# dflemin3/approxposterior

Measured on AMD Instinct MI355X. Metric: GP-predict+acquisition candidates/sec (N_train, D fixed), higher is better.
Workload: dtype f64

## Files before the change

approxposterior_amd/_lib.py:

```python
import ctypes
import os

_HERE = os.path.dirname(os.path.abspath(__file__))
LIB_PATH = os.path.join(_HERE, "csrc", "libapgp.so")
ABI_VERSION = 8
MAX_DIM = 32
MAX_FANTASY = 32
MAX_DRAWS = 32
MAX_FEATURES = 65536
MAX_REFS = 4096
INTEGRATED_MAX_DIM = 16

UTIL_AGP, UTIL_BAPE, UTIL_JONES, UTIL_NONE = 0, 1, 2, 3
UTIL_NEG_MEAN = 4
NM_MAX_RESTARTS = 4096
NM_MAX_FEV = 1 << 20
NM_STEPS = {1: "reflect", 2: "expand", 3: "reflect_exp", 4: "contract_out", 5: "contract_in",
            6: "shrink_out", 7: "shrink_in", 8: "maxfev"}
PRUNE_ROWS_SPLIT, PRUNE_ROWS_SIGNED = 0, 1
GMM_EM, GMM_SCORE, GMM_KMEANS = 0, 1, 2
GMM_MAX_COMP = 16
IMP_BLOCK = 256
IMP_MAX_BLOCKS = 2048

# ... 34 lines not shown

class HmcOptions(ctypes.Structure):
    _fields_ = [("eps", ctypes.c_double), ("jitter", ctypes.c_double), ("nleap", ctypes.c_int32),
                ("g_rows", ctypes.c_int32), ("iteration0", ctypes.c_int64), ("mass", ctypes.c_double * MAX_DIM)]

_P = ctypes.c_void_p
_I64 = ctypes.c_int64
_I32 = ctypes.c_int32
_F64 = ctypes.c_double
_KP = ctypes.POINTER(KernelStruct)

SIGNATURES = {
    "apgp_abi_version": (ctypes.c_int, []),
    "apgp_last_error": (ctypes.c_char_p, []),
    "apgp_npad": (_I64, [_I64]),
    "apgp_packed_linv_len": (_I64, [_I64]),
    "apgp_acquire_work_len": (_I64, [_I64, _I64]),
    "apgp_packed_train_len": (_I64, [_I64, _I32]),
    "apgp_trtri_work_len": (_I64, [_I64]),
    "apgp_grad_work_len": (_I64, [_I64]),
    "apgp_gram": (ctypes.c_int, [_P, _I64, _KP, _P, _I64, _P]),
    "apgp_kernel_cross": (ctypes.c_int, [_P, _I64, _P, _I64, _KP, _P, _I64, _P]),
    "apgp_potrf": (ctypes.c_int, [_P, _I64, _I64, _P, _F64, _P, _P, _P]),
    "apgp_logdet": (ctypes.c_int, [_P, _I64, _I64, _P, _P]),
    "apgp_fit_summary": (ctypes.c_int, [_P, _I64, _I64, _P, _P, _P, _P]),
    "apgp_nll_eval": (ctypes.c_int, [_P, _I64, _KP, _P, _F64, _P, _P, _P, _P, _P, _P]),
    "apgp_potrf_mode": (ctypes.c_int, [ctypes.c_int]),
    "apgp_potrf_fallbacks": (_I64, []),
    "apgp_potrf_backoff_skips": (_I64, []),
    "apgp_nll_side_batches": (_I64, []),
    "apgp_nll_eval_batch": (ctypes.c_int, [_P, _I64, _I64, _P, _P, _P, _P, _P, _P, _P, _P, _P]),
    "apgp_trsv": (ctypes.c_int, [_P, _I64, _I64, _P, _F64, ctypes.c_int, _P, _P, _P]),
    "apgp_trsv_ex": (ctypes.c_int, [_P, _I64, _I64, _P, _F64, ctypes.c_int, _P, _P, ctypes.c_int, _P]),
    "apgp_trsv_mode": (ctypes.c_int, [ctypes.c_int]),
    "apgp_append_diag": (ctypes.c_int, [_P, _P, _F64, _P, _I64, _P]),
    "apgp_winv_apply_work_len": (_I64, [_I64]),
    "apgp_winv_apply": (ctypes.c_int, [_P, _I64, _I64, _P, _F64, ctypes.c_int, _P, _P, _P, _P]),
    "apgp_trtri_pack": (ctypes.c_int, [_P, _I64, _I64, _P, _P, _P, _P]),
    "apgp_pack_train": (ctypes.c_int, [_P, _P, _I64, _KP, _P, _P]),
    "apgp_acquire": (ctypes.c_int, [_P, _I64, _I64, _P, _P, _I64, _KP, _F64, _I32,
                                    ctypes.POINTER(_F64), ctypes.POINTER(_F64), _P,
                                    _F64, _F64, _P, _P, _P, _P, _P, _P]),
    "apgp_packed_lsolve_len": (_I64, [_I64]),
    "apgp_pack_lsolve": (ctypes.c_int, [_P, _I64, _I64, _P, _P]),
    "apgp_acquire_solve": (ctypes.c_int, [_P, _I64, _I64, _P, _P, _I64, _KP, _F64, _I32,
                                          ctypes.POINTER(_F64), ctypes.POINTER(_F64), _P,
                                          _F64, _F64, _P, _P, _P, _P, _P, _P]),
    "apgp_set_sweep_prune": (ctypes.c_int, [ctypes.c_int]),
    "apgp_get_sweep_prune": (ctypes.c_int, []),
    "apgp_set_seed_rowsplit": (ctypes.c_int, [ctypes.c_int]),
    "apgp_get_seed_rowsplit": (ctypes.c_int, []),
    "apgp_set_seed_park": (ctypes.c_int, [ctypes.c_int]),
    "apgp_get_seed_park": (ctypes.c_int, []),
    "apgp_set_seed_first": (ctypes.c_int, [ctypes.c_int]),
    "apgp_get_seed_first": (ctypes.c_int, []),
    "apgp_set_seed_parts": (ctypes.c_int, [ctypes.c_int]),
    "apgp_get_seed_parts": (ctypes.c_int, []),
    "apgp_sweep_prune_counts_offset": (_I64, [_I64, _I64]),
    "apgp_sweep_prune_select": (ctypes.c_int, [_P, _I64, _P, _P, _F64, _P, _P]),
    "apgp_prune_bounds": (ctypes.c_int, [_P, _I64, _P, _I64, _KP, _F64, _I32, ctypes.POINTER(_F64), ctypes.POINTER(_F64),
                                         _P, _F64, _F64, ctypes.c_int, _P, _P]),
    "apgp_sweep_prune_seeds": (ctypes.c_int, [_P, _I64, _P, _P, _P]),
    "apgp_prune_rows_len": (_I64, [_I64, _I32]),
    "apgp_pack_prune_rows": (ctypes.c_int, [_P, _I64, _KP, _P, _P]),
    "apgp_acquire_rows": (ctypes.c_int, [_P, _I64, _I64, _P, _P, _I64, _KP, _F64, _I32,
                                         ctypes.POINTER(_F64), ctypes.POINTER(_F64), _P,
                                         _F64, _F64, _P, _P, _P, _P, _P, _P, _P]),
    "apgp_acquire_solve_rows": (ctypes.c_int, [_P, _I64, _I64, _P, _P, _I64, _KP, _F64, _I32,
                                               ctypes.POINTER(_F64), ctypes.POINTER(_F64), _P,
                                               _F64, _F64, _P, _P, _P, _P, _P, _P, _P]),
    "apgp_prune_bounds_rows": (ctypes.c_int, [_P, _I64, _P, _I64, _KP, _F64, _I32, ctypes.POINTER(_F64),
                                              ctypes.POINTER(_F64), _P, _F64, _F64, ctypes.c_int, _P, _P, _P]),
    "apgp_prune_srows_len": (_I64, [_I64, _I32]),
    "apgp_pack_prune_srows": (ctypes.c_int, [_P, _I64, _KP, _P, _P]),
    "apgp_acquire_rows2": (ctypes.c_int, [_P, _I64, _I64, _P, _P, _I64, _KP, _F64, _I32,
                                          ctypes.POINTER(_F64), ctypes.POINTER(_F64), _P,
                                          _F64, _F64, _P, _P, _P, _P, _P, _P, _I32, _P]),
    "apgp_acquire_solve_rows2": (ctypes.c_int, [_P, _I64, _I64, _P, _P, _I64, _KP, _F64, _I32,
                                                ctypes.POINTER(_F64), ctypes.POINTER(_F64), _P,
                                                _F64, _F64, _P, _P, _P, _P, _P, _P, _I32, _P]),
    "apgp_prune_bounds_rows2": (ctypes.c_int, [_P, _I64, _P, _I64, _KP, _F64, _I32, ctypes.POINTER(_F64),
                                               ctypes.POINTER(_F64), _P, _F64, _F64, ctypes.c_int, _P, _P, _I32, _P, _P]),
    "apgp_acquire_fantasy_work_len": (_I64, [_I64]),
    "apgp_acquire_fantasy": (ctypes.c_int, [_P, _I64, _I64, _P, _I64, _KP, _P, _I64, _I32, _P, _I64,
                                            _P, _P, _P, _I32, ctypes.POINTER(_F64), ctypes.POINTER(_F64), _P,
                                            _F64, _F64, _P, _P, _P, _P]),
    "apgp_path_draws_work_len": (_I64, [_I64, _I32]),
    "apgp_path_draws_mode": (ctypes.c_int, [ctypes.c_int]),
    "apgp_path_draws": (ctypes.c_int, [_P, _I64, _I64, _P, _I64, _KP, _F64, _P, _P, _P, _P, _P, _I32, _I32,
                                       ctypes.POINTER(_F64), ctypes.POINTER(_F64), _P, _P, _P, _P, _P]),
    "apgp_integrated_work_len": (_I64, [_I64, _I32]),
    "apgp_integrated_mode": (ctypes.c_int, [ctypes.c_int]),
    "apgp_acquire_integrated": (ctypes.c_int, [_P, _I64, _I64, _P, _I64, _KP, _P, _I32, _P, _P, _P,
                                               ctypes.POINTER(_F64), ctypes.POINTER(_F64), _P, _P, _I64, _P, _P, _P, _P]),
    "apgp_predict1_work_len": (_I64, [_I64]),
    "apgp_predict1_host": (ctypes.c_int, [_P, _P, _I64, _KP, _F64, _P, _I64, _P, _I64, _P, _P, _P]),
    "apgp_nm_search_work_len": (_I64, [_I64, _I64]),
    "apgp_nm_search": (ctypes.c_int, [_P, _I64, _P, _I64, _KP, _F64, _P, _I64, _P, _I64,
                                      ctypes.POINTER(_F64), ctypes.POINTER(_F64), ctypes.POINTER(NmOptions),
                                      _P, _P, _P, _P, _P, _P, _P]),
    "apgp_predict_grad_work_len": (_I64, [_I64, _I64]),
    "apgp_predict_grad": (ctypes.c_int, [_P, _I64, _P, _I64, _KP, _F64, _P, _I64, _P, _I64, _I32,
                                         ctypes.POINTER(_F64), ctypes.POINTER(_F64), _F64, _F64,
                                         _P, _P, _P, _P, _P, _P, _P, _P]),
    "apgp_predict_mean": (ctypes.c_int, [_P, _I64, _P, _I64, _KP, _F64, _P, _P]),
    "apgp_predict_mean_host": (ctypes.c_int, [_P, _I64, _P, _I64, _KP, _F64, _P, _P, _P]),
# ... 78 lines not shown
```

approxposterior_amd/csrc/prune_mm32.h:

```cpp
#pragma once
#include <utility>

#ifndef PMM_G
#define PMM_G 4
#endif
#define PMM_ROWS 128
typedef float f32x16 __attribute__((ext_vector_type(16)));
typedef __bf16 bf16x8 __attribute__((ext_vector_type(8)));

struct PmmSlot { int e, pp, qp; };

template <int DPAD>
struct PmmShape {
    static constexpr int K = DPAD + 2;
    static constexpr int NS = 5 * DPAD + 4;
    static constexpr int NIS = (NS + 15) / 16, NI = NIS + 1;
    static constexpr int PITCH = 16 * NI + 8;
    static_assert(K <= 16, "the big products stand in one instruction");
    static constexpr int XPIECES = PMM_ROWS * PITCH / 8, APIECES = PMM_ROWS / 4, PIECES = XPIECES + APIECES;
    static constexpr PmmSlot slot(int i) {
        if (i >= 16 * NIS) return i - 16 * NIS < K ? PmmSlot{i - 16 * NIS, 0, 0} : PmmSlot{-1, 0, 0};
        if (i < 2 * DPAD) return PmmSlot{2 + i / 2, (i & 1) ? 2 : 0, (i & 1) ? 0 : 2};
        i -= 2 * DPAD;
        if (i < 2) return i == 0 ? PmmSlot{0, 2, 0} : PmmSlot{1, 0, 2};
// ... 153 lines not shown
        for (int j = 0; j < NW; ++j) {
            if (j < w) k += pos ? wp[b][j] : wn[b][j];
            base_p += wp[b][j];
            base_n += wn[b][j];
        }
        k += __popcll((pos ? mp : mn) & below);
        if (in) {
            float pe[DPAD + 2];
            double n2 = 0.0, b2 = 0.0;
#pragma unroll
            for (int d = 0; d < DPAD; ++d) {
                const double x = (d & 1) ? pre[d >> 1].y : pre[d >> 1].x;
                const double df = x - cen[d];
                b2 = fma(df, df, b2);
                const float bf = (float)(df * kappa);
                n2 = fma((double)bf, (double)bf, n2);
                pe[d + 2] = 2.0f * bf;
            }
            bm2 = fmax(bm2, b2);
            sal += fabs(alpha);
            pe[0] = -(float)n2;
            pe[1] = 1.0f;
            const long long r = pmm_srow((pos ? 0 : gp) + (k >> 4), (int)(k & 15));
            pmm_put_row<DPAD>(img + r / PMM_ROWS * (16ll * SH::PIECES), (int)(r % PMM_ROWS), pe, (float)alpha);
        }
    }
    for (long long r = tid; r < pmm_stiles(n) * PMM_ROWS; r += PR_THREADS) {
        const int rr = (int)(r & 31), s = (rr & 3) + 4 * (rr >> 3);
        const long long q = 2 * (r >> 5) + ((rr >> 2) & 1);
        const bool empty = q < gp ? 16 * q + s >= np : q < gp + gn ? 16 * (q - gp) + s >= nn : true;
        if (empty) {
            float pe[DPAD + 2];
#pragma unroll
            for (int d = 0; d < DPAD; ++d) pe[d + 2] = 0.0f;
            pe[0] = -0.0f;
            pe[1] = 1.0f;
            pmm_put_row<DPAD>(img + r / PMM_ROWS * (16ll * SH::PIECES), (int)(r % PMM_ROWS), pe, 0.0f);
        }
    }
    for (int o = 32; o > 0; o >>= 1) { bm2 = fmax(bm2, __shfl_xor(bm2, o)); sal += __shfl_xor(sal, o); }
    if (lane == 0) { wmax[w] = bm2; wsal[w] = sal; }
    __syncthreads();
    if (tid == 0) {
        sal = 0.0;
#pragma unroll
        for (int i = 0; i < NW; ++i) { bm2 = fmax(bm2, wmax[i]); sal += wsal[i]; }
        ((double*)rows)[0] = bm2;
        ((double*)rows)[1] = sal;
        ((long long*)rows)[2] = (gp + gn + 1) / 2;
        ((long long*)rows)[3] = 0;
    }
}

template <int DPAD, bool PRE = false, bool SGN = false>
__global__ __launch_bounds__(PR_THREADS, PMM_G <= 4 ? 2 : 1) void prune_bound_mm32_kernel(PruneArgs a) {
    static_assert(PRE || !SGN, "the sign-sorted rows come as a stream only");
    using SH = PmmShape<DPAD>;
    constexpr int XS = DPAD + 2;
    constexpr int K = SH::K, NI = SH::NI, PITCH = SH::PITCH, G = PMM_G;
    static_assert(PMM_G % 2 == 0 && PMM_ROWS == 32 * (PR_THREADS / 64), "one 32-row tile staged per wavefront");
    const double kappa = PR32_KAPPA;
    static_assert(SH::XPIECES * 8 == PMM_ROWS * PITCH && SH::APIECES * 4 == PMM_ROWS, "the stream's tile is the LDS image");
    constexpr int NB = PRE ? 2 : 1;
    __shared__ __attribute__((aligned(16))) __bf16 xt[NB * PMM_ROWS * PITCH];
    __shared__ __attribute__((aligned(16))) float at[NB * PMM_ROWS];
    __shared__ double wmax[PR_THREADS / 64], wsal[PR_THREADS / 64];
    const int tid = threadIdx.x, lane = tid & 63, w = tid >> 6, h = lane >> 5, l32 = lane & 31;
    const long long blk0 = ((long long)blockIdx.x * (PR_THREADS / 64) + w) * (G / 2);
    double cen[DPAD], c2 = 0.0;
#pragma unroll
    for (int d = 0; d < DPAD; ++d) { cen[d] = a.xs[d]; c2 = fma(cen[d], cen[d], c2); }
    const double cn = sqrt(c2);
    bf16x8 qop[G][NI];
    double an[G];
    bool adm[G];
#pragma unroll
    for (int g = 0; g < G; ++g) {
        const long long blk = blk0 + (g >> 1);
        const long long row = blk * SW_CAND + (g & 1) * 32 + l32;
        const bool live = blk < a.ncb && row < a.m;
        bool ok = live, has_nan = false;
        double a2 = 0.0, ce[DPAD];
#pragma unroll
        for (int d = 0; d < DPAD; ++d) {
            double v = 0.0;
            if (live && d < a.ndim) {
                v = a.T[row * a.ndim + d];
                if (a.has_box && !(v >= a.lo[d] && v <= a.hi[d])) ok = false;
                if (v != v) has_nan = true;
            }
            ce[d] = v * a.sc[d] - cen[d];
            a2 = fma(ce[d], ce[d], a2);
        }
        if (live && a.mask && a.mask[row] == 0) ok = false;
        adm[g] = ok && !has_nan;
        an[g] = sqrt(a2);
        const bool use = live && !has_nan && a2 <= 0x1p100;
        float q[K];
        double n2 = 0.0;
#pragma unroll
        for (int d = 0; d < DPAD; ++d) {
            q[d + 2] = use ? (float)(ce[d] * kappa) : 0.0f;
            n2 = fma((double)q[d + 2], (double)q[d + 2], n2);
        }
        q[0] = 1.0f;
        q[1] = -(float)n2;
        pmm_cand<DPAD>(qop[g], q, h, std::make_integer_sequence<int, NI>{});
    }
    double accm[G], accs[G], sal = 0.0, bm2 = 0.0;
#pragma unroll
    for (int g = 0; g < G; ++g) { accm[g] = 0.0; accs[g] = 0.0; }
    long long nrt = 0;
    if constexpr (SGN) nrt = ((const long long*)a.prune_rows)[2];
    const long long ntile = SGN ? (nrt + PMM_ROWS / 32 - 1) / (PMM_ROWS / 32) : (a.n + PMM_ROWS - 1) / PMM_ROWS;
    auto consume = [&](int xo, int ao, int nr) {
#pragma unroll 1
        for (int rt = 0; rt < (SGN ? nr : PMM_ROWS / 32); ++rt) {
            const __bf16* xr = xt + xo + (rt * 32 + l32) * PITCH + 8 * h;
            bf16x8 pop[NI];
#pragma unroll
            for (int t = 0; t < NI; ++t) pop[t] = *(const bf16x8*)(xr + 16 * t);
            float al[16];
#pragma unroll
            for (int q = 0; q < 4; ++q) *(f32x4*)(al + 4 * q) = *(const f32x4*)(at + ao + rt * 32 + 8 * q + 4 * h);
            auto product = [&](int g) {
                f32x16 c = {0.0f, 0.0f, 0.0f, 0.0f, 0.0f, 0.0f, 0.0f, 0.0f, 0.0f, 0.0f, 0.0f, 0.0f, 0.0f, 0.0f, 0.0f, 0.0f};
#pragma unroll
                for (int t = 0; t < NI; ++t) c = __builtin_amdgcn_mfma_f32_32x32x16_bf16(pop[t], qop[g][t], c, 0, 0, 0);
                return c;
            };
            f32x16 cur = product(0);
#pragma unroll
            for (int g = 0; g < G; ++g) {
                f32x16 nxt = cur;
                if (g + 1 < G) nxt = product(g + 1);
                float ps = 0.0f, pS = 0.0f;
#pragma unroll
                for (int r = 0; r < 16; ++r) {
                    const float k = __builtin_amdgcn_exp2f(cur[r]);
                    ps = fmaf(k, al[r], ps);
                    if constexpr (!SGN) pS = fmaf(k, fabsf(al[r]), pS);
                }
                accm[g] += (double)ps;
                accs[g] += (double)(SGN ? fabsf(ps) : pS);
                cur = nxt;
            }
        }
    };
    if constexpr (PRE) {
        typedef unsigned int u32x4 __attribute__((ext_vector_type(4)));
        constexpr int NPC = SH::PIECES, NL = (NPC + PR_THREADS - 1) / PR_THREADS;
        const u32x4* img = (const u32x4*)((const unsigned char*)a.prune_rows + (SGN ? PMM_SHDR : 16));
        u32x4 pre[NL];
        auto fetch = [&](long long ti) {
            const u32x4* src = img + ti * NPC;
#pragma unroll
            for (int j = 0; j < NL; ++j) {
                const int e = tid + j * PR_THREADS;
                pre[j] = src[e < NPC ? e : NPC - 1];
            }
        };
        auto put = [&](int b) {
            u32x4* xd = (u32x4*)(xt + b * PMM_ROWS * PITCH);
            u32x4* ad = (u32x4*)(at + b * PMM_ROWS);
#pragma unroll
            for (int j = 0; j < NL; ++j) {
                const int e = tid + j * PR_THREADS;
                if ((j + 1) * PR_THREADS <= SH::XPIECES || e < SH::XPIECES) xd[e] = pre[j];
                else if (e < NPC) ad[e - SH::XPIECES] = pre[j];
            }
        };
        fetch(0);
        put(0);
        __syncthreads();
        for (long long ti = 0; ti < ntile; ++ti) {
            const int b = (int)(ti & 1);
            fetch(ti + 1 < ntile ? ti + 1 : ntile - 1);
            const long long left = nrt - ti * (PMM_ROWS / 32);
            consume(b * PMM_ROWS * PITCH, b * PMM_ROWS, left < PMM_ROWS / 32 ? (int)left : PMM_ROWS / 32);
            put(b ^ 1);
            __syncthreads();
        }
        bm2 = ((const double*)a.prune_rows)[0];
        sal = ((const double*)a.prune_rows)[1];
    } else {
        const bool stager = h == 0;
        const int srow = w * 32 + l32;
        f64x2 pre[XS / 2];
        auto fetch = [&](long long ti) {
            const f64x2* src = (const f64x2*)(a.xs + (ti * PMM_ROWS + srow) * XS);
#pragma unroll
            for (int i = 0; i < XS / 2; ++i) pre[i] = stager ? src[i] : f64x2{0.0, 0.0};
        };
        fetch(0);
        for (long long ti = 0; ti < ntile; ++ti) {
            if (stager) {
                const bool in = ti * PMM_ROWS + srow < a.n;
                float pe[K];
                double n2 = 0.0, b2 = 0.0;
#pragma unroll
                for (int d = 0; d < DPAD; ++d) {
                    const double x = (d & 1) ? pre[d >> 1].y : pre[d >> 1].x;
                    const double df = x - cen[d];
                    b2 = fma(df, df, b2);
                    const float bf = in ? (float)(df * kappa) : 0.0f;
                    n2 = fma((double)bf, (double)bf, n2);
                    pe[d + 2] = 2.0f * bf;
                }
                if (in) { bm2 = fmax(bm2, b2); sal += fabs(pre[DPAD / 2].x); }
                pe[0] = -(float)n2;
                pe[1] = 1.0f;
                pmm_store_row<DPAD>(xt + srow * PITCH, pe, std::make_integer_sequence<int, 2 * NI>{});
                at[srow] = in ? (float)pre[DPAD / 2].x : 0.0f;
            }
            __syncthreads();
            if (ti + 1 < ntile) fetch(ti + 1);
            consume(0, 0, PMM_ROWS / 32);
            __syncthreads();
        }
        for (int o = 32; o > 0; o >>= 1) { bm2 = fmax(bm2, __shfl_xor(bm2, o)); sal += __shfl_xor(sal, o); }
        if (lane == 0) { wmax[w] = bm2; wsal[w] = sal; }
        __syncthreads();
        sal = 0.0;
#pragma unroll
        for (int i = 0; i < PR_THREADS / 64; ++i) { bm2 = fmax(bm2, wmax[i]); sal += wsal[i]; }
    }
    const double bn = sqrt(bm2);
    const double u32 = 0x1p-24, eps = 0x1p-53;
    const double sa = sal * (1.0 + 0x1p-16);
    double bb = INFINITY, bbe = INFINITY;
#pragma unroll
    for (int g = 0; g < G; ++g) {
        const double sm = accm[g] + __shfl_xor(accm[g], 32);
// ... 18 lines not shown
```

approxposterior_amd/csrc/sweep.hip:

```cpp
#include "apgp_common.h"
#include "mma16.h"
#include "scratch.h"
#include "util_value.h"
#include <mutex>
#include <stdlib.h>
#include <string.h>

#define SW_ROWS APGP_ROW_BLOCK
#define SW_KC APGP_K_CHUNK
#define SW_TILE (SW_ROWS * SW_KC)
#define SW_CAND 64
#define SW_GRID 256
#define SW_BCH 1024
typedef unsigned int u32x4 __attribute__((ext_vector_type(4)));
#ifndef SW_KAUX
#define SW_KAUX 0
#endif

struct SweepArgs {
    const double* T;
    const double* linv;
    const double* xs;
    const unsigned char* mask;
    double* mu;
// ... 1099 lines not shown
            hipLaunchKernelGGL((sweep2_kernel<DPAD, true, 2, LIST>), dim3(grid), dim3(S2_THREADS), lds, s, a);
        else
            hipLaunchKernelGGL((sweep2_kernel<DPAD, false, 2, LIST>), dim3(grid), dim3(S2_THREADS), lds, s, a);
    } else if (solve) {
        if (a.lin_coef != 0.0)
            hipLaunchKernelGGL((sweep2_kernel<DPAD, true, 1, LIST>), dim3(grid), dim3(S2_THREADS), lds, s, a);
        else
            hipLaunchKernelGGL((sweep2_kernel<DPAD, false, 1, LIST>), dim3(grid), dim3(S2_THREADS), lds, s, a);
    } else if (a.lin_coef != 0.0)
        hipLaunchKernelGGL((sweep2_kernel<DPAD, true, 0, LIST>), dim3(grid), dim3(S2_THREADS), lds, s, a);
    else
        hipLaunchKernelGGL((sweep2_kernel<DPAD, false, 0, LIST>), dim3(grid), dim3(S2_THREADS), lds, s, a);
}

template <int DPAD>
static int launch_sweep(const SweepArgs& a0, hipStream_t s, bool solve) {
    const int rc = s2_prepare_device<DPAD>();
    if (rc != 0) return rc;
    SweepArgs a = a0;
    const long long ncb = (a.m + SW_CAND - 1) / SW_CAND;
    const int nrb2 = s2_nrb(a.n);
    a.nrb = nrb2;
    long long rest = ncb % SW_GRID;
    if (solve || nrb2 < 2 || rest > S2_SPLIT_MAX || a.sp_q == NULL) rest = 0;
    const long long full = ncb - rest;
    if (full > 0) {
        a.blk_begin = 0; a.blk_end = full; a.split = 0;
        s2_launch<DPAD, false>(a, s, solve, (unsigned)(full < SW_GRID ? full : SW_GRID));
    }
    if (rest > 0) {
        a.blk_begin = full; a.blk_end = ncb; a.split = 1;
        a.ncache = 0;
        a.kslot_bytes = SW_BCH * 8;
        s2_launch<DPAD, false>(a, s, solve, (unsigned)(rest * nrb2));
        hipLaunchKernelGGL(sweep_finish_kernel, dim3((unsigned)rest), dim3(64), 0, s, a);
    }
    return 0;
}

static int g_seed_rowsplit = -1;

extern "C" int apgp_set_seed_rowsplit(int v) {
    return __atomic_exchange_n(&g_seed_rowsplit, v < 0 ? -1 : v, __ATOMIC_RELAXED);
}

extern "C" int apgp_get_seed_rowsplit(void) { return __atomic_load_n(&g_seed_rowsplit, __ATOMIC_RELAXED); }

static int g_seed_park = 1;

extern "C" int apgp_set_seed_park(int v) { return __atomic_exchange_n(&g_seed_park, v != 0 ? 1 : 0, __ATOMIC_RELAXED); }

extern "C" int apgp_get_seed_park(void) { return __atomic_load_n(&g_seed_park, __ATOMIC_RELAXED); }

#define S2_SEED_FIRST 4
static int g_seed_first = -1;

extern "C" int apgp_set_seed_first(int v) {
    return __atomic_exchange_n(&g_seed_first, v < 1 ? -1 : (v > 16 ? 16 : v), __ATOMIC_RELAXED);
}

extern "C" int apgp_get_seed_first(void) { return __atomic_load_n(&g_seed_first, __ATOMIC_RELAXED); }

static int g_seed_parts = -1;

extern "C" int apgp_set_seed_parts(int v) {
    return __atomic_exchange_n(&g_seed_parts, (v == 8 || v == 4 || v == 2 || v == 1) ? v : -1, __ATOMIC_RELAXED);
}

extern "C" int apgp_get_seed_parts(void) { return __atomic_load_n(&g_seed_parts, __ATOMIC_RELAXED); }

static long long seed_launch_cost(int nrb, int cap, int n, int j0, int lg, bool parked) {
    static const int gen[4] = {S2P_WHOLE_GEN, S2P_HALF_GEN, S2P_PAIR2_GEN, S2P_PAIR1_GEN};
    static const int park[4] = {S2P_WHOLE_PARK, S2P_HALF_PARK, S2P_PAIR2_PARK, S2P_PAIR1_PARK};
    long long load[SW_GRID] = {0};
    const int nitem = s2_nitems(nrb, j0, n, lg);
    long long last = 0;
    for (int i = 0; i < nitem; ++i) {
        int jb = 0, h = -1;
        s2_row_item(i, nrb, j0, n, lg, jb, h);
        const int kind = h >= 0 ? lg : (n - S2_ROWS * jb <= S2_ROWS / 2 ? 1 : 0);
        const int nkc = s2_nkc_of(jb, n), nre = S2_CPB * jb < nkc ? S2_CPB * jb : nkc;
        const long long c = parked ? (long long)gen[kind] * (nkc - nre) + (long long)park[kind] * nre
                                   : (long long)s2_part_cost(kind) * nkc;
        for (int k = 0; k < cap; ++k) {
            int best = 0;
            for (int q = 1; q < SW_GRID; ++q)
                if (load[q] < load[best]) best = q;
            load[best] += c;
            if (load[best] > last) last = load[best];
        }
    }
    return last;
}

struct SeedPlan { int j0, lg; long long cost; };
static SeedPlan seed_plan(int nrb, int cap, int n, bool parked) {
    const int v = apgp_get_seed_rowsplit(), fp = apgp_get_seed_parts();
    const int flg = fp == 8 ? 0 : fp == 4 ? 1 : fp == 2 ? 2 : fp == 1 ? 3 : -1;
    struct Memo { int nrb, cap, n, parked, v, flg; SeedPlan plan; };
    static std::mutex mu;
    static Memo memo[8];
    static int nmemo = 0, next = 0;
    std::lock_guard<std::mutex> g(mu);
    for (int i = 0; i < nmemo; ++i) {
        const Memo& e = memo[i];
        if (e.nrb == nrb && e.cap == cap && e.n == n && e.parked == (int)parked && e.v == v && e.flg == flg) return e.plan;
// ... 558 lines not shown
    return old;
}

extern "C" int apgp_get_sweep_prune(void) { return __atomic_load_n(&g_sweep_prune, __ATOMIC_RELAXED); }

static inline long long pr_ncb(int64_t m) { return (m + SW_CAND - 1) / SW_CAND; }
static inline long long s2_work_len(int64_t m, int64_t n) {
    const long long ncb = pr_ncb(m);
    const long long slots = ncb < SW_GRID ? ncb : SW_GRID;
    return 2 * ncb + slots * s2_ncache(n) * SW_BCH + 2 * (long long)S2_SPLIT_MAX * SW_CAND * s2_nrb(n);
}

extern "C" int64_t apgp_sweep_prune_counts_offset(int64_t m, int64_t n) {
    if (m < 1 || n < 1 || m > APGP_MAX_M || n > APGP_MAX_N) return -1;
    return s2_work_len(m, n) + 2 * pr_ncb(m) + PR_SEED;
}

extern "C" int apgp_sweep_prune_select(const double* bmin, int64_t ncb, const int64_t* seeds, int64_t* counts,
                                       double tau, int64_t* list, void* stream) {
    APGP_CHECK_ARG(bmin && seeds && counts && list, "null pointer");
    APGP_CHECK_ARG(ncb >= 1 && ncb <= APGP_MAX_M / SW_CAND, "ncb >= 1 required");
    hipLaunchKernelGGL(prune_select_kernel, dim3(1), dim3(1024), 0, (hipStream_t)stream, bmin, (long long)ncb,
                       (const long long*)seeds, (long long*)counts, (const double*)NULL, tau, (long long*)list,
                       (long long*)NULL);
    APGP_CHECK_LAUNCH();
    return 0;
}

static inline bool pr_rows_kind_ok(const void* prune_rows, int rows_kind) {
    return rows_kind == APGP_PRUNE_ROWS_SPLIT || (rows_kind == APGP_PRUNE_ROWS_SIGNED && prune_rows != NULL);
}

template <class Kern>
static PruneArgs pr_args(const double* T, int64_t m, const double* xs, int64_t n, const uint8_t* mask, const Kern& kern,
                         double mean, int32_t kind, const double* lo, const double* hi, double zeta, double ybest,
                         double* bmin, double* part_u, long long* part_i, const void* prune_rows, int rows_kind) {
    PruneArgs p;
    p.T = T; p.xs = xs; p.mask = mask; p.bmin = bmin; p.part_u = part_u; p.part_i = part_i;
    p.m = m; p.ncb = pr_ncb(m); p.n = n;
    p.kind = kind; p.mean = mean; p.zeta = zeta; p.ybest = ybest;
    apgp_fill_kernel(p, kern);
    apgp_fill_box(p, p.ndim, lo, hi);
    p.blk_list = NULL; p.blk_count = NULL; p.est = NULL; p.prune_rows = prune_rows; p.rows_kind = rows_kind;
    return p;
}

template <int DPAD>
static void launch_bound(const PruneArgs& p, hipStream_t s, bool coarse) {
    auto grid_of = [&](int cpt) { return dim3((unsigned)((p.ncb + (PR_THREADS / 64) * cpt - 1) / ((PR_THREADS / 64) * cpt))); };
    const dim3 grid = grid_of(coarse ? pr32_cpt(DPAD) : PR_CPT);
    if (coarse) {
        if constexpr (DPAD <= 8) {
            const dim3 mm_grid = grid_of(PMM_G / 2);
            if (p.prune_rows && p.rows_kind == APGP_PRUNE_ROWS_SIGNED)
                hipLaunchKernelGGL((prune_bound_mm32_kernel<DPAD, true, true>), mm_grid, dim3(PR_THREADS), 0, s, p);
            else if (p.prune_rows)
                hipLaunchKernelGGL((prune_bound_mm32_kernel<DPAD, true>), mm_grid, dim3(PR_THREADS), 0, s, p);
            else
                hipLaunchKernelGGL((prune_bound_mm32_kernel<DPAD, false>), mm_grid, dim3(PR_THREADS), 0, s, p);
            hipLaunchKernelGGL((prune_bound32_kernel<DPAD, true>), grid, dim3(PR_THREADS), 0, s, p);
        } else {
            hipLaunchKernelGGL((prune_bound32_kernel<DPAD, false>), grid, dim3(PR_THREADS), 0, s, p);
        }
    } else if (p.blk_list)
        hipLaunchKernelGGL((prune_bound_kernel<DPAD, true>), grid, dim3(PR_THREADS), 0, s, p);
    else
        hipLaunchKernelGGL((prune_bound_kernel<DPAD, false>), grid, dim3(PR_THREADS), 0, s, p);
}

template <int DPAD>
static int launch_pruned(const SweepArgs& a, hipStream_t s, bool solve, void* part, const void* prune_rows,
                         int rows_kind) {
    const int rc = s2_prepare_device<DPAD>();
    if (rc != 0) return rc;
    const long long ncb = pr_ncb(a.m);
    double* bmin = (double*)part + s2_work_len(a.m, a.n);
    long long* list = (long long*)(bmin + ncb);
    long long* seeds = list + ncb;
    long long* counts = seeds + PR_SEED;
    const bool coarse = a.lin_coef == 0.0;
    PruneArgs p = pr_args(a.T, a.m, a.xs, a.n, a.mask, a, a.mean, a.kind, a.has_box ? a.lo : NULL, a.has_box ? a.hi : NULL,
                          a.zeta, a.ybest, bmin, a.part_u, a.part_i, prune_rows, rows_kind);
    if (coarse) p.est = (double*)(counts + 8);
    launch_bound<DPAD>(p, s, coarse);
    hipLaunchKernelGGL(prune_seed_kernel, dim3(1), dim3(1024), 0, s, coarse ? (const double*)p.est : (const double*)bmin, ncb,
                       seeds, counts);
    if (solve || s2_nrb(a.n) < 2 || a.sp_q == NULL) (void)hipMemsetAsync(counts + 4, 0, sizeof(long long), s);
    launch_sweep_list<DPAD>(a, s, solve, seeds, counts, ncb < PR_SEED ? ncb : PR_SEED, PR_SEED, true);
    hipLaunchKernelGGL(prune_select_kernel, dim3(1), dim3(1024), 0, s, bmin, ncb, seeds, counts, a.part_u, 0.0, list,
                       counts + 3);
    if (coarse) {
        p.blk_list = list; p.blk_count = counts + 3;
        launch_bound<DPAD>(p, s, false);
        hipLaunchKernelGGL(prune_select_kernel, dim3(1), dim3(1024), 0, s, bmin, ncb, seeds, counts, a.part_u, 0.0, list,
                           (long long*)NULL);
    }
    launch_sweep_list<DPAD>(a, s, solve, list, counts + 1, ncb, S2_SPLIT_MAX);
    return 0;
}

static_assert(S2_PRUNE_WORDS == PR_SEED + 8, "the fold inputs start behind the seed numbers and the counters");
static inline long long pr_work_len(int64_t m, int64_t n) {
    return s2_work_len(m, n) - 2ll * S2_SPLIT_MAX * SW_CAND * s2_nrb(n) + s2_fold_off(s2_nrb(n), pr_ncb(m));
}

extern "C" int64_t apgp_acquire_work_len(int64_t m, int64_t n) {
    if (m < 1 || n < 1) return 0;
// ... 566 lines not shown
```

approxposterior_amd/gp.py:

```python

import collections
import ctypes
import math
from operator import is_

import numpy as np
from numpy.linalg import LinAlgError
from scipy.linalg import solve_triangular

from . import _lib
from .george_extras import GeorgeExtras

__all__ = ["GP", "ExpSquaredKernel", "ConstantKernel", "Product", "ConstantModel",
           "kernels", "UTILITY_KINDS", "sobolSample"]

UTILITY_KINDS = {"agp": _lib.UTIL_AGP, "bape": _lib.UTIL_BAPE, "jones": _lib.UTIL_JONES}
SEARCH_KINDS = dict(UTILITY_KINDS, negmean=_lib.UTIL_NEG_MEAN)
NM_OPTIONS = ("adaptive", "maxiter", "maxfev", "xatol", "fatol")


def nm_coefficients(ndim, adaptive):
    if adaptive:
        dim = float(ndim)
        return 1.0, 1 + 2 / dim, 0.75 - 1 / (2 * dim), 1 - 1 / dim
# ... 326 lines not shown
            raise ValueError("Z (R, D), b (R,), W (S, R) and Wl (S, D) do not fit together")
        self.ks = gp._kernel_struct()
        self.mean = float(gp.mean.value)
        self._key, self._x = (gp._factor_key(), self.mean), gp._x

    def _check_current(self):
        gp = self.gp
        if not gp.computed or gp._x is not self._x or (gp._factor_key(), float(gp.mean.value)) != self._key:
            raise RuntimeError("these draws belong to a factor the GP no longer holds: call sample_paths again")

    def _call(self, t, bounds, mask, idx_offset, with_f):
        gp = self.gp
        self._check_current()
        lo, hi = _box(bounds, gp.kernel.ndim)
        T = gp._candidates(t)
        mask_d = mask if hasattr(mask, "data_ptr") else gp._mask(mask, T.shape[0])
        if mask_d is not None and (tuple(mask_d.shape) != (T.shape[0],) or str(mask_d.dtype) != "torch.uint8"):
            raise ValueError("a device mask must be a (M,) uint8 tensor")
        if T.shape[0] == 0:
            return np.empty((self.size, 0)), np.full(self.size, -1, dtype=np.int64), np.full(self.size, np.inf)
        return gp._path_call(T, self.ks, self.mean, self, self.V, lo, hi, mask_d, idx_offset, with_f)

    def evaluate(self, t):
        F = self._call(t, None, None, 0, True)[0]
        return F if isinstance(F, np.ndarray) else F.cpu().numpy()

    def argmax(self, t, bounds=None, mask=None, idx_offset=0):
        _, idx, u = self._call(t, bounds, mask, idx_offset, False)
        return idx, -u



class GP(GeorgeExtras):

    def __init__(self, kernel=None, fit_kernel=True, mean=None, fit_mean=None,
                 white_noise=None, fit_white_noise=None, solver=None, device=None,
                 **kwargs):
        if kernel is None:
            raise ValueError("a kernel is required")
        self.kernel = kernel
        self.mean = _as_model(mean, 0.0)
        self.white_noise = _as_model(white_noise, np.log(1.25e-12))
        self.fit_mean = bool(fit_mean)
        self.fit_white_noise = bool(fit_white_noise)
        self._device_arg = device
        self.variance_mode = None
        self.extend_max_rows = None
        self.sweep_prune = None
        self.seed_rowsplit = None
        self.seed_park = None
        self.seed_first = None
        self.seed_parts = None
        self.prune_signed = True
        self.sweep_prune_stats = False
        self.last_prune_counts = None
        self._computed = False
        self._x = None
        self._yerr2 = 0.0
        self._nllMemo = None
        self._rt_cache = None
        self._queries = None
        self._x_d = None
        self._mean_work = None
        self._p1_work = None
        self._imp_work = None
        self._pimp_work = None
        self._pg_work = None
        self._nll_scratch = None
        self._nll_stream = None
        self._batch = None
        self._replays = {}
        self._reset_device_state()

    def _reset_device_state(self):
        self._L = None
        self._L_store = None
        self._ld = None
        self._nll_owned = False
        self._alpha_y = None
        self._alpha_mean = None
        self._y_d = None
        self._ztz_host = None
        self._z = None
        self._alpha = None
        self._packed = None
        self._packed_solve = None
        self._work = None
        self._xs = None
        self._prune_rows = None
        self._prune_srows = None
        self._xs_key = None
        for key in ("nll", "one", "mean", "pgrad"):
            self._replays.pop(key, None)
        self.cond_estimate = None
        self.log_determinant = None

    def _rt(self):
        if self._rt_cache is not None:
            return self._rt_cache
        import torch
        lib = _lib.load()
        if not torch.cuda.is_available():
            raise _lib.ApgpError("no MI355X visible: approxposterior_amd has no CPU fallback")
        dev = self._device_arg
        if dev is None:
            dev = torch.device("cuda", torch.cuda.current_device())
# ... 691 lines not shown
            p0 = out.data_ptr()
            with_u = kid != _lib.UTIL_NONE
            args = [T.data_ptr(), m, self._xs.data_ptr(), n, ctypes.byref(ks), float(self.mean.value), *inv, kid,
                    lo, hi, float(zeta), float(np.max(y)),
                    p0, p0 + 8 * m, p0 + 16 * m if with_u else None, p0 + 24 * m, p0 + 8 * m * (3 + D),
                    p0 + 8 * m * (3 + 2 * D) if with_u else None, self._pg_work.data_ptr(), st]
            _lib.check(lib.apgp_predict_grad(*args), "apgp_predict_grad")
            if host_point:
                self._replays["pgrad"] = _Replay(
                    lib.apgp_predict_grad, args, dev.index, st.value or 0, y, (self._xs, self._pg_work, factor),
                    self._queries, data=((kid, bkey, float(zeta), self.mean.value), torch, T, out))
            if return_device:
                return self._pgrad_split(out, m, D, kid)
            return self._pgrad_split(out.cpu().numpy(), m, D, kid)

    @staticmethod
    def _pgrad_split(out, m, D, kid):
        mu, var, u = out[:m], out[m:2 * m], out[2 * m:3 * m]
        dmu, dvar, du = (out[m * (3 + j * D):m * (3 + (j + 1) * D)].reshape(m, D) for j in range(3))
        if kid == _lib.UTIL_NONE:
            return mu, var, dmu, dvar
        return u, du, mu, var

    def _sweep(self, y, T, kind_id, lo=None, hi=None, mask_d=None, zeta=0.01, idx_offset=0,
               with_mu=False, with_var=False, with_u=False):
        torch, dev, lib = self._rt()
        y = self._check_dimensions(y)
        n, m = len(self._x), T.shape[0]
        ks = self._kernel_struct()
        use_solve = not self._trust_inverse()
        with self._on(torch, dev):
            st = self._stream(torch)
            if use_solve:
                self._ensure_lsolve()
            else:
                self._ensure_linv()
            self._ensure_xs(y)
            f64 = dict(dtype=torch.float64, device=dev)
            mu, var, u = (torch.empty(m, **f64) if keep else None for keep in (with_mu, with_var, with_u))
            part = torch.empty(max(int(lib.apgp_acquire_work_len(m, n)), 2), **f64)
            best = torch.empty(2, **f64)
            ev = getattr(self, "kernel_events", None)
            if ev is not None:
                e0 = torch.cuda.Event(enable_timing=True)
                e0.record()
            args = (self._xs.data_ptr(), n, ctypes.byref(ks), float(self.mean.value), kind_id, lo, hi, _ptr(mask_d),
                    float(zeta), float(np.max(y)), _ptr(mu), _ptr(var), _ptr(u), part.data_ptr(), best.data_ptr(),
                    *self._prune_stream(), st)
            prune_was = None if self.sweep_prune is None else lib.apgp_set_sweep_prune(int(self.sweep_prune))
            rowsplit_was = None if self.seed_rowsplit is None else lib.apgp_set_seed_rowsplit(int(self.seed_rowsplit))
            park_was = None if self.seed_park is None else lib.apgp_set_seed_park(int(self.seed_park))
            first_was = None if self.seed_first is None else lib.apgp_set_seed_first(int(self.seed_first))
            parts_was = None if self.seed_parts is None else lib.apgp_set_seed_parts(int(self.seed_parts))
            try:
                if use_solve:
                    _lib.check(lib.apgp_acquire_solve_rows2(T.data_ptr(), m, int(idx_offset),
                                                            self._packed_solve.data_ptr(), *args), "apgp_acquire_solve_rows2")
                else:
                    _lib.check(lib.apgp_acquire_rows2(T.data_ptr(), m, int(idx_offset), self._packed.data_ptr(), *args),
                               "apgp_acquire_rows2")
            finally:
                if prune_was is not None:
                    lib.apgp_set_sweep_prune(prune_was)
                if rowsplit_was is not None:
                    lib.apgp_set_seed_rowsplit(rowsplit_was)
                if park_was is not None:
                    lib.apgp_set_seed_park(park_was)
                if first_was is not None:
                    lib.apgp_set_seed_first(first_was)
                if parts_was is not None:
                    lib.apgp_set_seed_parts(parts_was)
            if self.sweep_prune_stats and kind_id != _lib.UTIL_NONE and mu is None and var is None and u is None:
                off = int(lib.apgp_sweep_prune_counts_offset(m, n))
                self.last_prune_counts = part[off:off + 5].view(torch.int64).clone()
            if ev is not None:
                e1 = torch.cuda.Event(enable_timing=True)
                e1.record()
                ev.append((e0, e1))
        return _Swept(best, mu, var, u)

    def acquire(self, y, t, kind, bounds=None, mask=None, zeta=0.01, return_all=False,
                idx_offset=0, device_record=False):
        if not self.computed:
            raise RuntimeError("ERROR: Need to compute GP before using it!")
        kind_id = UTILITY_KINDS[str(kind).lower()]
        if device_record and return_all:
            raise ValueError("device_record returns the arg-min record only")
        torch, dev, _ = self._rt()
        lo, hi = _box(bounds, self.kernel.ndim)
        T = self._candidates(t)
        mask_d = self._mask(mask, T.shape[0])
        y = self._check_dimensions(y)
        if T.shape[0] == 0:
            if device_record:
                return torch.tensor([int(np.float64(np.inf).view(np.int64)), -1], dtype=torch.int64, device=dev)
            return (-1, float("inf")) + ((np.empty(0),) * 3 if return_all else ())
        s = self._sweep(y, T, kind_id, lo, hi, mask_d, zeta, idx_offset, with_mu=return_all, with_var=return_all,
                        with_u=return_all)
        if device_record:
            return s.best.view(torch.int64)
        if not return_all:
            return _best_record(s.best)
        return _best_record(s.best) + (s.u.cpu().numpy(), s.mu.cpu().numpy(), s.var.cpu().numpy())

    def prune_bounds(self, y, t, kind, coarse=True, bounds=None, mask=None, zeta=0.01):
        if not self.computed:
            raise RuntimeError("ERROR: Need to compute GP before using it!")
        kind_id = UTILITY_KINDS[str(kind).lower()]
        torch, dev, lib = self._rt()
        lo, hi = _box(bounds, self.kernel.ndim)
        T = self._candidates(t)
        m = T.shape[0]
        mask_d = self._mask(mask, m)
        y = self._check_dimensions(y)
        ks = self._kernel_struct()
        with self._on(torch, dev):
            self._ensure_xs(y)
            bmin = torch.empty((m + 63) // 64, dtype=torch.float64, device=dev)
            _lib.check(lib.apgp_prune_bounds_rows2(T.data_ptr(), m, self._xs.data_ptr(), len(self._x), ctypes.byref(ks),
                                                   float(self.mean.value), kind_id, lo, hi, _ptr(mask_d), float(zeta),
                                                   float(np.max(y)), int(bool(coarse)), bmin.data_ptr(),
                                                   *self._prune_stream(), None, self._stream(torch)),
                       "apgp_prune_bounds_rows2")
        return bmin.cpu().numpy()

    def nelder_mead_search(self, y, starts, kind, bounds=None, zeta=0.01, options=None, trace=False):
        try:
            kid = SEARCH_KINDS[str(kind).lower()]
        except KeyError:
            raise ValueError("kind must be one of %s" % sorted(SEARCH_KINDS))
        opts = dict(options or {})
        unknown = sorted(set(opts) - set(NM_OPTIONS))
        if unknown:
            raise ValueError("the device Nelder-Mead search does not take the option(s) %s (it takes %s)"
                             % (unknown, ", ".join(NM_OPTIONS)))
        if not self.computed:
            raise RuntimeError("ERROR: Need to compute GP before using it!")
        y = self._check_dimensions(y)
        D = self.kernel.ndim
        lo, hi = _box(bounds, D)
        X0 = np.ascontiguousarray(np.asarray(starts, dtype=np.float64).reshape(-1, D))
        R = len(X0)
        if not 1 <= R <= _lib.NM_MAX_RESTARTS:
            raise ValueError("between 1 and %d restarts per call" % _lib.NM_MAX_RESTARTS)
        rho, chi, psi, sigma = nm_coefficients(D, bool(opts.get("adaptive", False)))
        maxiter, maxfev = nm_limits(D, opts.get("maxiter"), opts.get("maxfev"))
        if not (1 <= maxiter <= _lib.NM_MAX_FEV and 1 <= maxfev <= _lib.NM_MAX_FEV):
            raise ValueError("maxiter and maxfev must lie between 1 and %d" % _lib.NM_MAX_FEV)
        opt = _lib.NmOptions(kind=kid, maxiter=maxiter, maxfev=maxfev, reserved=0, zeta=float(zeta),
                             ybest=float(np.max(y)), xatol=float(opts.get("xatol", 1e-4)),
                             fatol=float(opts.get("fatol", 1e-4)), rho=rho, chi=chi, psi=psi, sigma=sigma)
        torch, dev, lib = self._rt()
        n = len(self._x)
        ks = self._kernel_struct()
        use_solve = not self._trust_inverse()
        with self._on(torch, dev):
            st = self._stream(torch)
            if not use_solve:
                self._ensure_linv()
            self._ensure_xs(y)
            f64 = dict(dtype=torch.float64, device=dev)
            i32 = dict(dtype=torch.int32, device=dev)
            starts_d = torch.from_numpy(X0).to(dev)
            x_out = torch.empty((R, D), **f64)
            f_out = torch.empty(R, **f64)
            stats = torch.zeros((R, 3), **i32)
            work = torch.empty(int(lib.apgp_nm_search_work_len(R, n)), **f64)
            tr = torch.empty(R * maxfev * (D + 3), **f64) if trace else None
            steps = torch.zeros(R * maxiter, **i32) if trace else None
            inv, _ = self._variance_operand(use_solve)
            _lib.check(lib.apgp_nm_search(starts_d.data_ptr(), R, self._xs.data_ptr(), n, ctypes.byref(ks),
                                          float(self.mean.value), *inv, lo, hi, ctypes.byref(opt),
                                          x_out.data_ptr(), f_out.data_ptr(), stats.data_ptr(),
                                          _ptr(tr), _ptr(steps), work.data_ptr(), st),
                       "apgp_nm_search")
            x = x_out.cpu().numpy()
# ... 887 lines not shown
```

include/apgp.h:

```cpp
#ifndef APGP_H
#define APGP_H

#include <stddef.h>
#include <stdint.h>

#ifdef __cplusplus
extern "C" {
#endif

#define APGP_ABI_VERSION 8
#define APGP_MAX_DIM 32
#define APGP_ROW_BLOCK 512
#define APGP_K_CHUNK 16
#define APGP_CAND_BLOCK 64

#define APGP_UTIL_AGP 0
#define APGP_UTIL_BAPE 1
#define APGP_UTIL_JONES 2
#define APGP_UTIL_NONE 3
#define APGP_UTIL_NEG_MEAN 4

typedef struct apgp_kernel {
    int32_t ndim;
    int32_t lin_order;
// ... 41 lines not shown
int64_t apgp_potrf_backoff_skips(void);

int64_t apgp_nll_side_batches(void);
int apgp_nll_eval_batch(const double* X, int64_t n, int64_t batch,
                        const apgp_kernel_t* kerns , const double* y,
                        const double* means , double* K, double* z,
                        int32_t* info_dev, double* out5_dev, double* out5_host ,
                        void* stream);

int apgp_trsv(const double* L, int64_t n, int64_t ldl, const double* b, double shift,
              int trans, double* x, double* sumsq, void* stream);
int apgp_trsv_mode(int multi_launch);
int apgp_trsv_ex(const double* L, int64_t n, int64_t ldl, const double* b, double shift,
                 int trans, double* x, double* sumsq, int mode, void* stream);

int apgp_append_diag(double* ljj, const double* ss, double kdiag, int32_t* info_dev, int64_t order,
                     void* stream);

int64_t apgp_winv_apply_work_len(int64_t n);
int apgp_winv_apply(const double* winv, int64_t ldw, int64_t n, const double* b, double shift,
                    int trans, double* x, double* sumsq, double* work, void* stream);

int apgp_trtri_pack(const double* L, int64_t n, int64_t ldl, double* work,
                    double* packed, double* winv_dense, void* stream);

int apgp_pack_train(const double* X, const double* alpha, int64_t n,
                    const apgp_kernel_t* kern , double* xs, void* stream);

int64_t apgp_acquire_work_len(int64_t m, int64_t n);
int apgp_acquire(const double* T, int64_t m, int64_t idx_offset,
                 const double* packed_linv, const double* xs, int64_t n,
                 const apgp_kernel_t* kern , double mean, int32_t kind,
                 const double* lo , const double* hi ,
                 const uint8_t* mask, double zeta, double ybest,
                 double* mu, double* var, double* u,
                 void* part, apgp_best_t* best, void* stream);

int64_t apgp_packed_lsolve_len(int64_t n);
int apgp_pack_lsolve(const double* L, int64_t n, int64_t ldl, double* packed, void* stream);
int apgp_acquire_solve(const double* T, int64_t m, int64_t idx_offset,
                       const double* packed_lsolve, const double* xs, int64_t n,
                       const apgp_kernel_t* kern , double mean, int32_t kind,
                       const double* lo , const double* hi ,
                       const uint8_t* mask, double zeta, double ybest,
                       double* mu, double* var, double* u,
                       void* part, apgp_best_t* best, void* stream);

int apgp_set_sweep_prune(int v);
int apgp_get_sweep_prune(void);
int apgp_set_seed_rowsplit(int v);
int apgp_get_seed_rowsplit(void);
int apgp_set_seed_park(int v);
int apgp_get_seed_park(void);
int apgp_set_seed_first(int v);
int apgp_get_seed_first(void);
int apgp_set_seed_parts(int v);
int apgp_get_seed_parts(void);
int64_t apgp_sweep_prune_counts_offset(int64_t m, int64_t n);
int apgp_sweep_prune_select(const double* bmin, int64_t ncb, const int64_t* seeds, int64_t* counts,
                            double tau, int64_t* list, void* stream);
int apgp_prune_bounds(const double* T, int64_t m, const double* xs, int64_t n,
                      const apgp_kernel_t* kern , double mean, int32_t kind,
                      const double* lo , const double* hi , const uint8_t* mask,
                      double zeta, double ybest, int coarse, double* bmin_out, void* stream);
int apgp_sweep_prune_seeds(const double* bmin, int64_t ncb, int64_t* seeds, int64_t* counts, void* stream);

int64_t apgp_prune_rows_len(int64_t n, int32_t ndim);
int apgp_pack_prune_rows(const double* xs, int64_t n, const apgp_kernel_t* kern , void* rows, void* stream);
int apgp_acquire_rows(const double* T, int64_t m, int64_t idx_offset,
                      const double* packed_linv, const double* xs, int64_t n,
                      const apgp_kernel_t* kern , double mean, int32_t kind,
                      const double* lo , const double* hi ,
                      const uint8_t* mask, double zeta, double ybest,
                      double* mu, double* var, double* u,
                      void* part, apgp_best_t* best, const void* prune_rows, void* stream);
int apgp_acquire_solve_rows(const double* T, int64_t m, int64_t idx_offset,
                            const double* packed_lsolve, const double* xs, int64_t n,
                            const apgp_kernel_t* kern , double mean, int32_t kind,
                            const double* lo , const double* hi ,
                            const uint8_t* mask, double zeta, double ybest,
                            double* mu, double* var, double* u,
                            void* part, apgp_best_t* best, const void* prune_rows, void* stream);
int apgp_prune_bounds_rows(const double* T, int64_t m, const double* xs, int64_t n,
                           const apgp_kernel_t* kern , double mean, int32_t kind,
                           const double* lo , const double* hi , const uint8_t* mask,
                           double zeta, double ybest, int coarse, double* bmin_out, const void* prune_rows,
                           void* stream);

#define APGP_PRUNE_ROWS_SPLIT 0
#define APGP_PRUNE_ROWS_SIGNED 1
int64_t apgp_prune_srows_len(int64_t n, int32_t ndim);
int apgp_pack_prune_srows(const double* xs, int64_t n, const apgp_kernel_t* kern , void* rows, void* stream);
int apgp_acquire_rows2(const double* T, int64_t m, int64_t idx_offset,
                       const double* packed_linv, const double* xs, int64_t n,
                       const apgp_kernel_t* kern , double mean, int32_t kind,
                       const double* lo , const double* hi ,
                       const uint8_t* mask, double zeta, double ybest,
                       double* mu, double* var, double* u,
                       void* part, apgp_best_t* best, const void* prune_rows, int32_t rows_kind, void* stream);
int apgp_acquire_solve_rows2(const double* T, int64_t m, int64_t idx_offset,
                             const double* packed_lsolve, const double* xs, int64_t n,
                             const apgp_kernel_t* kern , double mean, int32_t kind,
                             const double* lo , const double* hi ,
                             const uint8_t* mask, double zeta, double ybest,
                             double* mu, double* var, double* u,
                             void* part, apgp_best_t* best, const void* prune_rows, int32_t rows_kind, void* stream);
// ... 212 lines not shown
```

Before: 920.7 million.

## Software-pipeline MFMA products with exp2 accumulation in signed prune-bound kernel

Adds a pipelined row-consume path to the signed-stream prune bound kernel. It overlaps the next group's MFMA product with the exp2/FMA reduction of the current one, double-buffers the LDS row operands in registers, and moves the next tile's global fetch into the middle of the current tile's consume. The aim is to hide MFMA latency and load latency behind the transcendental work. The path is on by default through a runtime toggle. It raises register pressure at two-block occupancy and relies on scheduling barriers and asm fences.

New measurement: 975.6 million, median of 6. 1.06x the previous value.

```diff
diff --git a/approxposterior_amd/_lib.py b/approxposterior_amd/_lib.py
--- a/approxposterior_amd/_lib.py
+++ b/approxposterior_amd/_lib.py
@@ -110,6 +110,8 @@
     "apgp_get_seed_rowsplit": (ctypes.c_int, []),
     "apgp_set_seed_park": (ctypes.c_int, [ctypes.c_int]),
     "apgp_get_seed_park": (ctypes.c_int, []),
+    "apgp_set_prune_pipe": (ctypes.c_int, [ctypes.c_int]),
+    "apgp_get_prune_pipe": (ctypes.c_int, []),
     "apgp_set_seed_first": (ctypes.c_int, [ctypes.c_int]),
     "apgp_get_seed_first": (ctypes.c_int, []),
     "apgp_set_seed_parts": (ctypes.c_int, [ctypes.c_int]),
diff --git a/approxposterior_amd/csrc/prune_mm32.h b/approxposterior_amd/csrc/prune_mm32.h
--- a/approxposterior_amd/csrc/prune_mm32.h
+++ b/approxposterior_amd/csrc/prune_mm32.h
@@ -229,9 +229,11 @@
     }
 }
 
-template <int DPAD, bool PRE = false, bool SGN = false>
+template <int DPAD, bool PRE = false, bool SGN = false, bool PIPE = false>
 __global__ __launch_bounds__(PR_THREADS, PMM_G <= 4 ? 2 : 1) void prune_bound_mm32_kernel(PruneArgs a) {
     static_assert(PRE || !SGN, "the sign-sorted rows come as a stream only");
+    static_assert((PRE && SGN) || !PIPE, "the pipelined row loop is written for the sign-sorted stream");
+    static_assert(!PIPE || (PMM_G == 4 && PMM_ROWS == 128), "consume_pipe: four groups alternate two accumulator tiles, four matrix tiles alternate two register sets");
     using SH = PmmShape<DPAD>;
     constexpr int XS = DPAD + 2;
     constexpr int K = SH::K, NI = SH::NI, PITCH = SH::PITCH, G = PMM_G;
@@ -324,6 +326,90 @@
             }
         }
     };
+    [[maybe_unused]] f32x16 c0, c1;
+    [[maybe_unused]] bf16x8 pA[NI], pB[NI];
+    [[maybe_unused]] float alA[16], alB[16];
+    auto consume_pipe = [&](int xo, int ao, int nr, bool first, bool last, auto&& fetch_next)
+                            __attribute__((always_inline)) {
+        auto rdp = [&](int rt, bf16x8 (&p)[NI]) __attribute__((always_inline)) {
+            const __bf16* xr = xt + xo + (rt * 32 + l32) * PITCH + 8 * h;
+#pragma unroll
+            for (int t = 0; t < NI; ++t) p[t] = *(const bf16x8*)(xr + 16 * t);
+        };
+        auto rda = [&](int rt, float (&al)[16]) __attribute__((always_inline)) {
+#pragma unroll
+            for (int q = 0; q < 4; ++q) *(f32x4*)(al + 4 * q) = *(const f32x4*)(at + ao + rt * 32 + 8 * q + 4 * h);
+        };
+        auto step = [&](auto next, f32x16& cc, const float (&al)[16], int g, f32x16& cn, const bf16x8 (&pn)[NI],
+                        int gn) __attribute__((always_inline)) {
+            constexpr bool NEXT = decltype(next)::value;
+            f32x16 c = {0.0f, 0.0f, 0.0f, 0.0f, 0.0f, 0.0f, 0.0f, 0.0f, 0.0f, 0.0f, 0.0f, 0.0f, 0.0f, 0.0f, 0.0f, 0.0f};
+            float ps = 0.0f;
+#pragma unroll
+            for (int t = 0; t < NI; ++t) {
+                if constexpr (NEXT) {
+                    if (t) asm volatile("" : "+v"(c));
+                    c = __builtin_amdgcn_mfma_f32_32x32x16_bf16(pn[t], qop[gn][t], c, 0, 0, 0);
+                    asm volatile("" : "+v"(c));
+                    asm volatile("" : "+v"(cc));
+                }
+#pragma unroll
+                for (int r = 16 * t / NI; r < 16 * (t + 1) / NI; ++r) {
+                    const float k = __builtin_amdgcn_exp2f(cc[r]);
+                    ps = fmaf(k, al[r], ps);
+                }
+                if constexpr (NEXT) {
+                    asm volatile("" : "+v"(ps));
+                    __builtin_amdgcn_sched_barrier(0);
+                }
+            }
+            accm[g] += (double)ps;
+            accs[g] += (double)fabsf(ps);
+            if constexpr (NEXT) cn = c;
+        };
+        const std::true_type under{};
+        const std::false_type alone{};
+        auto product0 = [&](const bf16x8 (&p)[NI]) __attribute__((always_inline)) {
+            f32x16 c = {0.0f, 0.0f, 0.0f, 0.0f, 0.0f, 0.0f, 0.0f, 0.0f, 0.0f, 0.0f, 0.0f, 0.0f, 0.0f, 0.0f, 0.0f, 0.0f};
+#pragma unroll
+            for (int t = 0; t < NI; ++t) c = __builtin_amdgcn_mfma_f32_32x32x16_bf16(p[t], qop[0][t], c, 0, 0, 0);
+            c0 = c;
+        };
+        auto tile = [&](auto more, int rt, const bf16x8 (&p)[NI], const float (&al)[16], bf16x8 (&pn)[NI], float (&aln)[16])
+                        __attribute__((always_inline)) {
+            constexpr bool MORE = decltype(more)::value;
+            if constexpr (MORE) rdp(rt + 1, pn);
+            step(under, c0, al, 0, c1, p, 1);
+            step(under, c1, al, 1, c0, p, 2);
+            step(under, c0, al, 2, c1, p, 3);
+            if constexpr (MORE) {
+                rda(rt + 1, aln);
+                step(under, c1, al, G - 1, c0, pn, 0);
+            }
+        };
+        if (nr == PMM_ROWS / 32) {
+            rdp(0, pA);
+            rda(0, alA);
+            if (first) product0(pA);
+            else step(under, c1, alB, G - 1, c0, pA, 0);
+            tile(under, 0, pA, alA, pB, alB);
+            tile(under, 1, pB, alB, pA, alA);
+            tile(under, 2, pA, alA, pB, alB);
+            if (!last) fetch_next();
+            tile(alone, 3, pB, alB, pA, alA);
+            if (last) step(alone, c1, alB, G - 1, c0, pA, 0);
+        } else {
+#pragma unroll 1
+            for (int rt = 0; rt < nr; ++rt) {
+                rdp(rt, pA);
+                rda(rt, alA);
+                if (rt == 0 && !first) step(under, c1, alB, G - 1, c0, pA, 0);
+                else product0(pA);
+                tile(alone, rt, pA, alA, pB, alB);
+                step(alone, c1, alA, G - 1, c0, pA, 0);
+            }
+        }
+    };
     if constexpr (PRE) {
         typedef unsigned int u32x4 __attribute__((ext_vector_type(4)));
         constexpr int NPC = SH::PIECES, NL = (NPC + PR_THREADS - 1) / PR_THREADS;
@@ -352,10 +438,16 @@
         __syncthreads();
         for (long long ti = 0; ti < ntile; ++ti) {
             const int b = (int)(ti & 1);
-            fetch(ti + 1 < ntile ? ti + 1 : ntile - 1);
+            if constexpr (!PIPE) fetch(ti + 1 < ntile ? ti + 1 : ntile - 1);
             const long long left = nrt - ti * (PMM_ROWS / 32);
-            consume(b * PMM_ROWS * PITCH, b * PMM_ROWS, left < PMM_ROWS / 32 ? (int)left : PMM_ROWS / 32);
-            put(b ^ 1);
+            if constexpr (PIPE) {
+                consume_pipe(b * PMM_ROWS * PITCH, b * PMM_ROWS, left < PMM_ROWS / 32 ? (int)left : PMM_ROWS / 32, ti == 0,
+                             ti + 1 == ntile, [&]() __attribute__((always_inline)) { fetch(ti + 1); });
+                if (ti + 1 < ntile) put(b ^ 1);
+            } else {
+                consume(b * PMM_ROWS * PITCH, b * PMM_ROWS, left < PMM_ROWS / 32 ? (int)left : PMM_ROWS / 32);
+                put(b ^ 1);
+            }
             __syncthreads();
         }
         bm2 = ((const double*)a.prune_rows)[0];
diff --git a/approxposterior_amd/csrc/sweep.hip b/approxposterior_amd/csrc/sweep.hip
--- a/approxposterior_amd/csrc/sweep.hip
+++ b/approxposterior_amd/csrc/sweep.hip
@@ -1175,6 +1175,12 @@
 
 extern "C" int apgp_get_seed_park(void) { return __atomic_load_n(&g_seed_park, __ATOMIC_RELAXED); }
 
+static int g_prune_pipe = 1;
+
+extern "C" int apgp_set_prune_pipe(int v) { return __atomic_exchange_n(&g_prune_pipe, v != 0 ? 1 : 0, __ATOMIC_RELAXED); }
+
+extern "C" int apgp_get_prune_pipe(void) { return __atomic_load_n(&g_prune_pipe, __ATOMIC_RELAXED); }
+
 #define S2_SEED_FIRST 4
 static int g_seed_first = -1;
 
@@ -1839,7 +1845,9 @@
     if (coarse) {
         if constexpr (DPAD <= 8) {
             const dim3 mm_grid = grid_of(PMM_G / 2);
-            if (p.prune_rows && p.rows_kind == APGP_PRUNE_ROWS_SIGNED)
+            if (p.prune_rows && p.rows_kind == APGP_PRUNE_ROWS_SIGNED && apgp_get_prune_pipe())
+                hipLaunchKernelGGL((prune_bound_mm32_kernel<DPAD, true, true, true>), mm_grid, dim3(PR_THREADS), 0, s, p);
+            else if (p.prune_rows && p.rows_kind == APGP_PRUNE_ROWS_SIGNED)
                 hipLaunchKernelGGL((prune_bound_mm32_kernel<DPAD, true, true>), mm_grid, dim3(PR_THREADS), 0, s, p);
             else if (p.prune_rows)
                 hipLaunchKernelGGL((prune_bound_mm32_kernel<DPAD, true>), mm_grid, dim3(PR_THREADS), 0, s, p);
diff --git a/approxposterior_amd/gp.py b/approxposterior_amd/gp.py
--- a/approxposterior_amd/gp.py
+++ b/approxposterior_amd/gp.py
@@ -402,6 +402,7 @@
         self.seed_first = None
         self.seed_parts = None
         self.prune_signed = True
+        self.prune_pipe = None
         self.sweep_prune_stats = False
         self.last_prune_counts = None
         self._computed = False
@@ -1199,6 +1200,7 @@
             park_was = None if self.seed_park is None else lib.apgp_set_seed_park(int(self.seed_park))
             first_was = None if self.seed_first is None else lib.apgp_set_seed_first(int(self.seed_first))
             parts_was = None if self.seed_parts is None else lib.apgp_set_seed_parts(int(self.seed_parts))
+            pipe_was = None if self.prune_pipe is None else lib.apgp_set_prune_pipe(int(self.prune_pipe))
             try:
                 if use_solve:
                     _lib.check(lib.apgp_acquire_solve_rows2(T.data_ptr(), m, int(idx_offset),
@@ -1217,6 +1219,8 @@
                     lib.apgp_set_seed_first(first_was)
                 if parts_was is not None:
                     lib.apgp_set_seed_parts(parts_was)
+                if pipe_was is not None:
+                    lib.apgp_set_prune_pipe(pipe_was)
             if self.sweep_prune_stats and kind_id != _lib.UTIL_NONE and mu is None and var is None and u is None:
                 off = int(lib.apgp_sweep_prune_counts_offset(m, n))
                 self.last_prune_counts = part[off:off + 5].view(torch.int64).clone()
@@ -1264,11 +1268,16 @@
         with self._on(torch, dev):
             self._ensure_xs(y)
             bmin = torch.empty((m + 63) // 64, dtype=torch.float64, device=dev)
-            _lib.check(lib.apgp_prune_bounds_rows2(T.data_ptr(), m, self._xs.data_ptr(), len(self._x), ctypes.byref(ks),
-                                                   float(self.mean.value), kind_id, lo, hi, _ptr(mask_d), float(zeta),
-                                                   float(np.max(y)), int(bool(coarse)), bmin.data_ptr(),
-                                                   *self._prune_stream(), None, self._stream(torch)),
-                       "apgp_prune_bounds_rows2")
+            pipe_was = None if self.prune_pipe is None else lib.apgp_set_prune_pipe(int(self.prune_pipe))
+            try:
+                _lib.check(lib.apgp_prune_bounds_rows2(T.data_ptr(), m, self._xs.data_ptr(), len(self._x), ctypes.byref(ks),
+                                                       float(self.mean.value), kind_id, lo, hi, _ptr(mask_d), float(zeta),
+                                                       float(np.max(y)), int(bool(coarse)), bmin.data_ptr(),
+                                                       *self._prune_stream(), None, self._stream(torch)),
+                           "apgp_prune_bounds_rows2")
+            finally:
+                if pipe_was is not None:
+                    lib.apgp_set_prune_pipe(pipe_was)
         return bmin.cpu().numpy()
 
     def nelder_mead_search(self, y, starts, kind, bounds=None, zeta=0.01, options=None, trace=False):
diff --git a/include/apgp.h b/include/apgp.h
--- a/include/apgp.h
+++ b/include/apgp.h
@@ -117,6 +117,8 @@
 int apgp_get_seed_rowsplit(void);
 int apgp_set_seed_park(int v);
 int apgp_get_seed_park(void);
+int apgp_set_prune_pipe(int v);
+int apgp_get_prune_pipe(void);
 int apgp_set_seed_first(int v);
 int apgp_get_seed_first(void);
 int apgp_set_seed_parts(int v);
```
